# sunshinnnn/DSMnet

Hardware: AMD Instinct MI355X
Metric: stereo pairs/sec forward, PSMNet D=192 384×1280, at 1/2/4/8 MI355X (higher is better)
Workload: dtype f32

## Files before the change

dsmnet_amd/_lib.py:

```python
import ctypes
import os

_HERE = os.path.dirname(os.path.abspath(__file__))
LIB_PATH = os.environ.get("DSM_LIB_PATH") or os.path.join(_HERE, "csrc", "libdsmnet_hip.so")

c_int, c_void_p, c_size_t = ctypes.c_int, ctypes.c_void_p, ctypes.c_size_t

DSM_OK = 0
DSM_F32 = 0
DSM_NCDHW, DSM_NDHWC = 0, 1
DSM_CONV_FP32_MFMA, DSM_CONV_COUT1_CHUNKED, DSM_CONV_TM_SHIFT, DSM_CONV_BLOCKS_SHIFT = 1, 2, 4, 16
DSM_CONV_NO_NSPLIT = 4
DSM_CONV_NO_ONCE = 8
DSM_CONV_KSPLIT_SHIFT = 8
DSM_PREC_F32, DSM_PREC_F16, DSM_PREC_F16X2 = 0, 1, 2
DSM_SIM_DOT, DSM_SIM_COSINE = 0, 1
DSM_CORR_BWD_NAIVE = 1


class Bn3dArgs(ctypes.Structure):
    _fields_ = [("y", c_void_p), ("residual", c_void_p), ("out", c_void_p), ("gamma", c_void_p),
                ("beta", c_void_p), ("running_mean", c_void_p), ("running_var", c_void_p),
                ("affine", c_void_p), ("workspace", c_void_p), ("gout", c_void_p), ("dy", c_void_p),
                ("dresidual", c_void_p), ("B", c_int), ("C", c_int),
                ("Dy", c_int), ("Hy", c_int), ("Wy", c_int), ("Dr", c_int), ("Hr", c_int), ("Wr", c_int),
                ("relu", c_int), ("momentum", ctypes.c_float), ("eps", ctypes.c_float),
                ("out_amax", c_void_p), ("dy_amax", c_void_p), ("dres_amax", c_void_p)]


class Conv3dArgs(ctypes.Structure):
    _fields_ = [("x", c_void_p), ("w_packed", c_void_p), ("scale", c_void_p),
                ("shift", c_void_p), ("residual", c_void_p), ("y", c_void_p),
                ("B", c_int), ("Cin", c_int), ("Cout", c_int),
                ("Di", c_int), ("Hi", c_int), ("Wi", c_int),
                ("Do", c_int), ("Ho", c_int), ("Wo", c_int),
                ("Dr", c_int), ("Hr", c_int), ("Wr", c_int),
                ("stride", c_int), ("transposed", c_int), ("relu", c_int),
                ("kd", c_int), ("k", c_int), ("dil", c_int),
                ("flags", c_int), ("precision", c_int), ("x_amax", c_void_p), ("y_amax", c_void_p),
                ("vol_virtual", c_int), ("vol_mask_left", c_int),
                ("workspace", c_void_p), ("workspace_bytes", c_size_t)]
# ... 135 lines not shown
    "dsm_conv_packed_weight_bytes": (ctypes.c_size_t, [c_int] * 4),
    "dsm_spp_branch_floats": (ctypes.c_size_t, [c_int] * 3),
    "dsm_spp_pool8": (c_int, [c_void_p] * 2 + [c_int] * 3 + [c_void_p]),
    "dsm_spp_branches": (c_int, [c_void_p] * 5 + [c_int] * 3 + [c_void_p]),
    "dsm_spp_concat": (c_int, [c_void_p] * 4 + [c_int] * 3 + [c_void_p] * 2),
    "dsm_warp_abs_error": (c_int, [c_void_p] * 4 + [c_int] * 6 + [ctypes.c_float, c_void_p]),
    "dsm_warp_abs_error_bwd": (c_int, [c_void_p] * 7 + [c_int] * 6 + [ctypes.c_float, c_void_p]),
    "dsm_decoder_cat_bwd": (c_int, [c_void_p] * 6 + [c_int] * 11 + [c_void_p]),
    "dsm_selfsup_workspace_floats": (c_size_t, [ctypes.POINTER(SelfsupItem), c_int]),
    "dsm_selfsup_fwd": (c_int, [ctypes.POINTER(SelfsupItem), c_int, c_int] + [c_void_p] * 4),
    "dsm_selfsup_bwd": (c_int, [ctypes.POINTER(SelfsupItem), c_int, c_int] + [c_void_p] * 4),
    "dsm_selfsup_ext_workspace_floats": (c_size_t, [ctypes.POINTER(SelfsupItem), c_int, c_int]),
    "dsm_selfsup_ext_fwd": (c_int, [ctypes.POINTER(SelfsupItem), ctypes.POINTER(SelfsupExt), c_int, c_int] + [c_void_p] * 4),
    "dsm_selfsup_ext_bwd": (c_int, [ctypes.POINTER(SelfsupItem), ctypes.POINTER(SelfsupExt), c_int, c_int] + [c_void_p] * 4),
    "dsm_selfsup_dyn_fwd": (c_int, [ctypes.POINTER(SelfsupItem), ctypes.POINTER(SelfsupExt), c_int, c_int] + [c_void_p] * 5),
    "dsm_selfsup_dyn_bwd": (c_int, [ctypes.POINTER(SelfsupItem), ctypes.POINTER(SelfsupExt), c_int, c_int] + [c_void_p] * 5),
    "dsm_suploss_workspace_floats": (c_size_t, [c_int] * 5),
    "dsm_suploss_fwd": (c_int, [ctypes.POINTER(SuplossItem), c_int, c_void_p, c_int, c_int, c_int, c_int] + [c_void_p] * 4),
    "dsm_suploss_bwd": (c_int, [ctypes.POINTER(SuplossItem), c_int, c_void_p, c_int, c_int, c_int] + [c_void_p] * 4),
    "dsm_stereo_metrics_workspace_bytes": (c_size_t, [c_int] * 3),
    "dsm_stereo_metrics": (c_int, [ctypes.POINTER(MetricsArgs), c_void_p]),
    "dsm_lr_check": (c_int, [ctypes.POINTER(LrcheckArgs), c_void_p]),
    "dsm_fill_background_workspace_bytes": (c_size_t, [c_int] * 3),
    "dsm_fill_background": (c_int, [c_void_p] * 4 + [c_int] * 3 + [c_void_p]),
    "dsm_disp_encode_workspace_bytes": (c_size_t, [c_int] * 3),
    "dsm_disp_encode": (c_int, [ctypes.POINTER(EncodeArgs), c_void_p]),
    "dsm_stereo_color": (c_int, [c_void_p, c_void_p, ctypes.POINTER(ColorRecord)] + [c_int] * 6 + [c_void_p]),
    "dsm_stereo_spatial": (c_int, [c_void_p, c_void_p, ctypes.POINTER(SpatialRecord)] + [c_int] * 8 + [c_void_p]),
    "dsm_stereo_spatial_raw": (c_int, [c_void_p, c_size_t, ctypes.POINTER(FrameSource), c_void_p,
                                       ctypes.POINTER(SpatialRecord)] + [c_int] * 8 + [c_void_p]),
    "dsm_stereo_spatial_raw_plan": (c_int, [c_void_p, c_size_t, ctypes.POINTER(FrameSource), c_void_p,
                                            ctypes.POINTER(SpatialRecord)] + [c_int] * 8),
    "dsm_concat_conv_fwd": (c_int, [c_void_p] * 5 + [c_size_t] + [c_void_p] * 2 + [c_int] * 9 + [c_void_p]),
}

_lib = None


class DsmnetHipError(RuntimeError):
    pass


def _bind_torch_hip_runtime():
    import torch
    hip = os.path.join(os.path.dirname(torch.__file__), "lib", "libamdhip64.so")
    if os.path.exists(hip):
        ctypes.CDLL(hip, mode=ctypes.RTLD_GLOBAL)


def load():
    global _lib
    if _lib is not None:
        return _lib
    if not os.path.exists(LIB_PATH):
        raise DsmnetHipError(
            "libdsmnet_hip.so not found at %s -- build it with "
            "`python -m dsmnet_amd.csrc.build` (there is no CPU fallback)" % LIB_PATH)
    _bind_torch_hip_runtime()
    lib = ctypes.CDLL(LIB_PATH)
    for name, (res, args) in SIGNATURES.items():
        fn = getattr(lib, name)
        fn.restype = res
        fn.argtypes = args
    if lib.dsm_abi_version() != 7:
        raise DsmnetHipError("libdsmnet_hip.so ABI version mismatch")
    _lib = lib
# ... 8 lines not shown
```

dsmnet_amd/blocks2d.py:

```python
import torch
import torch.nn as nn
import torch.nn.functional as F

from . import costvolume as cv
from . import blocks3d
from .folds import _bump_running_stats, _versions, fold_affine

_TRAIN_2D_MODE = __import__("os").environ.get("DSM_TRAIN_2D", "auto")
_FUSED_TRAIN_2D = _TRAIN_2D_MODE in ("auto", "fused", "conv")
_FUSED_TRAIN_2D_BN = _TRAIN_2D_MODE == "fused"
_TRAIN_2D_MIN_PIXELS = int(__import__("os").environ.get("DSM_TRAIN_2D_MIN_PIXELS", 65536)) if _TRAIN_2D_MODE == "auto" else 0


class own_kernels_only(object):

    def __enter__(self):
        global _TRAIN_2D_MIN_PIXELS, _FUSED_TRAIN_2D
        self.saved = (_TRAIN_2D_MIN_PIXELS, _FUSED_TRAIN_2D)
        _TRAIN_2D_MIN_PIXELS, _FUSED_TRAIN_2D = 0, True
        return self

    def __exit__(self, *exc):
        global _TRAIN_2D_MIN_PIXELS, _FUSED_TRAIN_2D
        _TRAIN_2D_MIN_PIXELS, _FUSED_TRAIN_2D = self.saved
# ... 56 lines not shown
    if not (cv.get_option("wide_conv2d_train") and isinstance(act, nn.ReLU) and isinstance(conv, nn.Conv2d) and
            x.is_cuda and x.dtype == torch.float32):
        return False
    k, s, d, p = conv.kernel_size, conv.stride, conv.dilation, conv.padding
    if k != (3, 3) or s[0] != s[1] or s[0] not in (1, 2) or d != (1, 1) or p != (1, 1) or conv.groups != 1:
        return False
    if conv.bias is None or conv.padding_mode != "zeros" or conv.weight.dtype != torch.float32:
        return False
    if conv.in_channels not in cv.WIDE2D_COUT or conv.out_channels not in cv.WIDE2D_COUT:
        return False
    B, _, H, W = x.shape
    Ho, Wo = (H - 1) // s[0] + 1, (W - 1) // s[0] + 1
    if W > 2032 or B * H * W >= 2 ** 20 or 4 * B * Ho * Wo * conv.out_channels >= 2 ** 31:
        return False
    return _wide_ok(conv, x)


class _Folded2d(object):
    def __init__(self):
        self.key = None
        self.packed = self.scale = self.shift = None

    def get(self, conv, bn, cin_padded):
        srcs = [conv.weight, conv.bias]
        if bn is not None:
            srcs += [bn.weight, bn.bias, bn.running_mean, bn.running_var]
        key = _versions(*srcs) + (cin_padded,)
        if key != self.key:
            with torch.no_grad():
                self.packed = cv.pack_conv2d_weight(conv.weight, cin_padded)
                self.scale, self.shift = fold_affine(conv.bias, bn, conv.out_channels, conv.weight.device)
            self.key = key
        return self.packed, self.scale, self.shift


def train_ok(conv, x):
    if not (_FUSED_TRAIN_2D and isinstance(conv, nn.Conv2d) and torch.is_tensor(x) and x.is_cuda and
            x.dtype == torch.float32 and conv.weight.dtype == torch.float32):
        return False
    k, s, d, p = conv.kernel_size, conv.stride, conv.dilation, conv.padding
    if k[0] != k[1] or s[0] != s[1] or d[0] != d[1] or p[0] != p[1] or conv.groups != 1:
        return False
    if conv.bias is not None or conv.padding_mode != "zeros" or p[0] != d[0] * (k[0] // 2):
        return False
    if x.shape[0] * ((x.shape[2] - 1) // s[0] + 1) * ((x.shape[3] - 1) // s[0] + 1) < _TRAIN_2D_MIN_PIXELS:
        return False
    return x.shape[1] == conv.in_channels and cv.conv2d_variant(conv.out_channels, s[0], k[0], d[0])


def _run_conv2d_autograd(conv, bn, x, residual, relu):
    y = cv.conv2d(x, conv.weight, conv.stride[0], conv.dilation[0])
    if (bn is not None and bn.training and _FUSED_TRAIN_2D_BN and blocks3d._FUSED_TRAIN_BN and
            y.shape[1] % 4 == 0 and y.shape[1] <= 256):
        momentum = bn.momentum if bn.momentum is not None else 0.1
        out = cv.bn_add_relu2d(y, bn.weight, bn.bias, residual,
                               bn.running_mean if bn.track_running_stats else None,
                               bn.running_var if bn.track_running_stats else None,
                               1 if relu else 0, momentum, bn.eps)
        if bn.num_batches_tracked is not None:
            bn.num_batches_tracked += 1
        _bump_running_stats(bn)
        return out
    if bn is not None:
        y = bn(y)
    if residual is not None:
        y = y + residual
    return F.relu(y) if relu else y


def run_conv2d(folded, conv, bn, x, residual=None, relu=False):
    training = bn is not None and bn.training
    if not training and not torch.is_grad_enabled() and fused_ok(conv, x):
        packed, scale, shift = folded.get(conv, bn, x.shape[1])
        return cv.conv2d_block(x, packed, conv.out_channels, scale, shift, residual,
                               stride=conv.stride[0], relu=1 if relu else 0,
                               k=conv.kernel_size[0], dilation=conv.dilation[0])
    if train_ok(conv, x):
        return _run_conv2d_autograd(conv, bn, x, residual, relu)
    if x.shape[1] != conv.in_channels:
        x = x[:, : conv.in_channels]
    y = conv(x)
    if bn is not None:
        y = bn(y)
    if residual is not None:
        y = y + residual
    return F.relu(y) if relu else y


def run_basicblock_layers(fold1, c1, b1, fold2, c2, b2, x, relu_after, skip=True):
    if b1 is None or b2 is None or c1.training or b1.training or b2.training or torch.is_grad_enabled():
        return None
    if not (fused_ok(c1, x) and fused_ok(c2, x) and c1.kernel_size[0] == 3 and c2.kernel_size[0] == 3 and
            c2.stride[0] == 1 and c2.dilation[0] == 1 and c2.in_channels == c2.out_channels == c1.out_channels and
            cv.basicblock2d_ok(x, c1.in_channels, c1.out_channels, c1.stride[0], c1.dilation[0])):
        return None
    p1, s1, h1 = fold1.get(c1, b1, x.shape[1])
    p2, s2, h2 = fold2.get(c2, b2, x.shape[1])
    return cv.basicblock2d(x, p1, s1, h1, p2, s2, h2, relu=relu_after, skip=skip)


def run_basicblock(cb1, cb2, x, downsample):
    if downsample is not None or not isinstance(cb1, ConvBN2d) or not isinstance(cb2, ConvBN2d):
        return None
    return run_basicblock_layers(cb1._folded, cb1[0], cb1[1], cb2._folded, cb2[0], cb2[1], x, False)

# ... 14 lines not shown
```

dsmnet_amd/costvolume.py:

```python
import collections
import ctypes
import functools
import os
import weakref

import torch

from . import _lib
from .folds import _versions

_CL3D = torch.channels_last_3d


class LaunchTimer(object):

    def __init__(self):
        self.records = []

    def start(self):
        ev = torch.cuda.Event(enable_timing=True)
        ev.record()
        return ev

    def stop(self, name, start, work):
# ... 446 lines not shown
            setattr(a, field, 16)
    buf = ctypes.create_string_buffer(96)
    rc = _lib.load().dsm_conv3d_plan(ctypes.byref(a), buf, 96)
    return rc, buf.value.decode()


_PRECISIONS = ("bf16x3", "fp32", "f16x2", "f16")


def _env_precision():
    v = os.environ.get("DSM_CONV_PRECISION", "")
    if v and v not in _PRECISIONS:
        raise ValueError("DSM_CONV_PRECISION must be one of %s, got %r" % (_PRECISIONS, v))
    return v or "f16x2"


def _env_flag(name, default):
    v = os.environ.get(name, "")
    if v not in ("", "0", "1"):
        raise ValueError("%s must be 0 or 1, got %r" % (name, v))
    return default if v == "" else v == "1"


_WIDE_CONV2D_DEFAULT = False

_OPTIONS = {"fuse_volume": True, "fuse_blocks": True, "conv_precision": _env_precision(), "conv_flags": 0,
            "separable_volume": _env_flag("DSM_SEPARABLE_VOLUME", True), "separable_flags": 0,
            "fused_supervised_loss": _env_flag("DSM_FUSED_SUP_LOSS", True),
            "wide_conv2d": _env_flag("DSM_WIDE_CONV2D", _WIDE_CONV2D_DEFAULT),
            "wide_conv2d_train": _env_flag("DSM_WIDE_CONV2D_TRAIN", False),
            "conv2d_k5": _env_flag("DSM_CONV2D_K5", False),
            "warp_train": _env_flag("DSM_WARP_TRAIN", False),
            "decoder_train": _env_flag("DSM_DECODER_TRAIN", False),
            "corr1d_tiled_bwd": False}


def set_option(name, value):
    if name == "conv_fp32":
        old = _OPTIONS["conv_precision"] == "fp32"
        _OPTIONS["conv_precision"] = "fp32" if value else "bf16x3"
        return old
    if name not in _OPTIONS:
        raise KeyError(name)
    old = _OPTIONS[name]
    if name == "conv_precision":
        if value not in _PRECISIONS:
            raise ValueError("conv_precision must be one of %s" % (_PRECISIONS,))
        _OPTIONS[name] = value
    else:
        _OPTIONS[name] = int(value) if name in ("conv_flags", "separable_flags") else bool(value)
    return old


def _mode(mode):
    return _OPTIONS["conv_precision"] if mode is None else mode


def _conv_flags(mode=None):
    return (_lib.DSM_CONV_FP32_MFMA if _mode(mode) == "fp32" else 0) | _OPTIONS["conv_flags"]


def get_option(name):
    if name == "conv_fp32":
        return _OPTIONS["conv_precision"] == "fp32"
    return _OPTIONS[name]

# ... 623 lines not shown
        if needs_amax():
            dy._dsm_amax = _ARENA.slot(y.device)
            a.dy_amax = dy._dsm_amax.data_ptr()
            if dres is not None:
                dres._dsm_amax = _ARENA.slot(y.device)
                a.dres_amax = dres._dsm_amax.data_ptr()
        with torch.cuda.device(y.device), _timed("bn3d_train_bwd_kernels", 4.0 * (3 * y.numel() + gout.numel())):
            rc = _lib.load().dsm_bn3d_train_bwd(ctypes.byref(a), _stream())
        _lib.check(rc, "dsm_bn3d_train_bwd")
        dbeta = ws[:C].float() if has_beta else None
        dgamma = ws[C:].float() if has_gamma else None
        return dy, dgamma, dbeta, dres, None, None, None, None, None


def bn_add_relu3d(y, gamma, beta, residual, running_mean, running_var, relu, momentum, eps):
    return BnAddRelu3dFunction.apply(y, gamma, beta, residual, running_mean, running_var, int(relu),
                                     float(momentum), float(eps))


def stage_images_nhwc16(left, right=None):
    _require_device("stage_images_nhwc16", left, right)
    left = left.contiguous()
    B, C, H, W = left.shape
    if right is not None:
        if tuple(right.shape) != tuple(left.shape):
            raise ValueError("stage_images_nhwc16: the two views differ in shape")
        right = right.contiguous()
    out = torch.empty(((1 if right is None else 2) * B, 16, H, W), device=left.device,
                      dtype=torch.float32, memory_format=_CL2D)
    with torch.cuda.device(left.device):
        rc = _lib.load().dsm_stage_images_nhwc16(_p(left), _p(right), _p(out), B, C, H, W, _stream())
    _lib.check(rc, "dsm_stage_images_nhwc16")
    return out


def conv2d_variant(cout, stride, k, dilation):
    if cout not in (32, 64, 128) or k not in (1, 3) or stride < 1 or dilation < 1:
        return False
    return _conv2d_variant(cout, stride, k, dilation, _mode(None), _conv_flags())


@functools.lru_cache(maxsize=None)
def _conv2d_variant(cout, stride, k, dilation, mode, flags):
    return _conv_plan(_conv2d_standin(1, 16, cout, 12, 40, stride, k, dilation, mode, flags))[0] == _lib.DSM_OK


def _wgrad2d(x_cl, g_cl, stride, dilation, label="conv2d_wgrad_kernel", mode=None):
    B, cx, Hx, Wx = x_cl.shape
    _, cg, Hg, Wg = g_cl.shape
    ws = torch.empty((cx // 32) * (cg // 32) * 9 * 1024, device=x_cl.device, dtype=torch.float32)
    dw = torch.empty((cg, cx, 3, 3), device=x_cl.device, dtype=torch.float32)
    prec, xa, ga = _wgrad_precision(x_cl, g_cl, mode)
    with torch.cuda.device(x_cl.device), _timed(label, 18.0 * cx * cg * B * Hg * Wg):
        rc = _lib.load().dsm_conv2d_wgrad(_p(x_cl), _p(g_cl), _p(ws), _p(dw), B, cx, cg, Hx, Wx,
                                          Hg, Wg, int(stride), int(dilation), _conv_flags(mode), prec,
                                          _p(xa), _p(ga), _stream())
    _lib.check(rc, "dsm_conv2d_wgrad")
    return dw


class Conv2dFunction(torch.autograd.Function):

    @staticmethod
    def forward(ctx, x, weight, stride, dilation):
        _require_device("Conv2dFunction", x, weight)
        cout, cin, k, _ = weight.shape
# ... 838 lines not shown
```

dsmnet_amd/csrc/build.py:

```python
import glob
import os
import subprocess
import sys
from concurrent.futures import ThreadPoolExecutor

HERE = os.path.dirname(os.path.abspath(__file__))
SOURCES = ["abi.hip", "corr1d.hip", "cost_volume.hip", "soft_argmin.hip", "conv3d.hip", "conv_f16.hip",
           "conv3d_bwd.hip", "bn3d.hip", "decoder.hip", "spp.hip", "warp.hip",
           "selfsup.hip", "color.hip", "spatial.hip", "frames.hip", "sepvol.hip", "suploss.hip", "relu_bwd.hip",
           "metrics.hip", "lrcheck.hip", "encode.hip"]
LIB = os.path.join(HERE, "libdsmnet_hip.so")
HIPCC = os.environ.get("HIPCC", "/opt/rocm/bin/hipcc")
FLAGS = ["--offload-arch=gfx950", "-O3", "-std=c++17", "-fPIC",
         "-Wall", "-Wno-unused-function"] + os.environ.get("HIPCC_EXTRA", "").split()


def _stale(out, deps):
    if not os.path.exists(out):
        return True
    t = os.path.getmtime(out)
    return any(os.path.getmtime(d) > t for d in deps)


def build(force=False, verbose=True, stamps=False):
    if stamps:
        lib = os.path.join(HERE, "libdsmnet_hip_stamps.so")
        srcs = [os.path.join(HERE, s) for s in SOURCES]
        extra = ["-DDSM_ABLATE=%s" % os.environ["DSM_ABLATE"]] if os.environ.get("DSM_ABLATE") else []
        cmd = [HIPCC] + FLAGS + ["-DDSM_STAMPS"] + extra + ["-shared", "-o", lib] + srcs
        print(" ".join(cmd), flush=True)
        subprocess.run(cmd, check=True)
        return lib
    hdrs = sorted(glob.glob(os.path.join(HERE, "*.hpp"))) + [os.path.join(HERE, "..", "..", "include", "dsmnet_hip.h")]
    srcs = [os.path.join(HERE, s) for s in SOURCES if os.path.exists(os.path.join(HERE, s))]
    objs = []
    jobs = []
    for s in srcs:
        o = s[:-4] + ".o"
        objs.append(o)
        if force or _stale(o, [s] + hdrs):
            jobs.append([HIPCC] + FLAGS + ["-c", s, "-o", o])

    def run(cmd):
# ... 18 lines not shown
```

dsmnet_amd/models/psmnet/stackhourglass.py:

```python
import math

import torch
import torch.nn as nn

from ... import costvolume as cv
from ...blocks3d import Chain3d, ConvBN3d
from .submodule import convbn_3d, disparityregression, feature_extraction


def myadd_3d(tensor1, tensor2):
    assert tensor1.dim() == 5
    d, h, w = (min(a, b) for a, b in zip(tensor1.shape[2:], tensor2.shape[2:]))
    return tensor1[:, :, :d, :h, :w] + tensor2[:, :, :d, :h, :w]


def _deconvbn_3d(cin, cout):
    return ConvBN3d(nn.ConvTranspose3d(cin, cout, kernel_size=3, padding=1, output_padding=1,
                                       stride=2, bias=False), nn.BatchNorm3d(cout))


class hourglass(nn.Module):
    def __init__(self, inplanes):
        super(hourglass, self).__init__()
        c = inplanes
# ... 19 lines not shown
        self.name = "psmnet"
        self.maxdisp = maxdisp
        self.align_corners = bool(align_corners)
        self.count_levels = 1
        self.feature_extraction = feature_extraction(align_corners=align_corners)
        relu = lambda: nn.ReLU(inplace=True)
        self.dres0 = Chain3d(convbn_3d(64, 32, 3, 1, 1), relu(), convbn_3d(32, 32, 3, 1, 1), relu())
        self.dres1 = Chain3d(convbn_3d(32, 32, 3, 1, 1), relu(), convbn_3d(32, 32, 3, 1, 1))
        self.dres2 = hourglass(32)
        self.dres3 = hourglass(32)
        self.dres4 = hourglass(32)
        for i in (1, 2, 3):
            setattr(self, "classif%d" % i, Chain3d(
                convbn_3d(32, 32, 3, 1, 1), relu(),
                nn.Conv3d(32, 1, kernel_size=3, padding=1, stride=1, bias=False)))
        self._init_weights()

    def _init_weights(self):
        for m in self.modules():
            if isinstance(m, (nn.Conv2d, nn.Conv3d)):
                fan = m.out_channels
                for k in m.kernel_size:
                    fan *= k
                m.weight.data.normal_(0, math.sqrt(2.0 / fan))
            elif isinstance(m, (nn.BatchNorm2d, nn.BatchNorm3d)):
                m.weight.data.fill_(1)
                m.bias.data.zero_()

    def features(self, left, right):
        if self.training:
            return self.feature_extraction(left), self.feature_extraction(right)
        fe = self.feature_extraction
        if left.is_cuda and not torch.is_grad_enabled() and left.shape[1] <= 16:
            both = fe(cv.stage_images_nhwc16(left, right), staged=True)
        else:
            both = self.feature_extraction(torch.cat([left, right], dim=0))
        self.__dict__["_both"] = both
        return (cv.carry_amax(both[: left.shape[0]], both), cv.carry_amax(both[left.shape[0]:], both))

    def regularise(self, cost):
        cost0 = self.dres0(cost)
        cost0 = self.dres1(cost0, residual=cost0)
        out1, pre1, post1 = self.dres2(cost0, None, None, skip=cost0)
        out2, pre2, post2 = self.dres3(out1, pre1, post1, skip=cost0)
        out3, pre3, post3 = self.dres4(out2, pre1, post2, skip=cost0)
        cost1 = self.classif1(out1)
        cost2 = self.classif2(out2, residual=cost1)
        cost3 = self.classif3(out3, residual=cost2)
        return cost1, cost2, cost3

    def forward(self, left, right, mode="train"):
        with cv.amax_scope(left.device):
            return self._forward(left, right)

    def head_cost(self, left, right):
        if self.training:
            raise RuntimeError("PSMNet.head_cost: eval mode only (call model.eval() first)")
        with cv.amax_scope(left.device):
            (_, _, cost3), size = self._head_costs(left, right)
        return cost3, size, False, self.align_corners, None

    def _forward(self, left, right):
        (cost1, cost2, cost3), size = self._head_costs(left, right)
        pred1 = cv.soft_argmin(cost1, size, align_corners=self.align_corners)
        pred2 = cv.soft_argmin(cost2, size, align_corners=self.align_corners)
        pred3 = cv.soft_argmin(cost3, size, align_corners=self.align_corners)
        return [0, 0, 0], [pred3, pred2, pred1]
# ... 13 lines not shown
```

dsmnet_amd/models/psmnet/submodule.py:

```python
import torch
import torch.nn as nn
import torch.nn.functional as F

from ... import blocks2d
from ... import costvolume as cv
from ...blocks2d import ConvBN2d, _Folded2d, run_conv2d, stage_image_nhwc16
from ...blocks3d import ConvBN3d
from ...folds import _versions, fold_affine

_SPP_MATMUL = __import__("os").environ.get("DSM_TRAIN_SPP", "matmul") != "interp"
_TRAIN_NHWC = __import__("os").environ.get("DSM_TRAIN_LAYOUT", "nchw") == "nhwc"


def convbn(in_planes, out_planes, kernel_size, stride, pad, dilation):
    del pad
    return ConvBN2d(
        nn.Conv2d(in_planes, out_planes, kernel_size=kernel_size, stride=stride,
                  padding=dilation, dilation=dilation, bias=False),
        nn.BatchNorm2d(out_planes))


def convbn_3d(in_planes, out_planes, kernel_size, stride, pad):
    conv = nn.Conv3d(in_planes, out_planes, kernel_size=kernel_size, padding=pad,
                     stride=stride, bias=False)
# ... 84 lines not shown
            return F.interpolate(y, size=size, mode="bilinear", align_corners=self.align_corners)
        key = (y.shape[2], y.shape[3], size[0], size[1], self.align_corners, y.device)
        cache = self.__dict__.setdefault("_up_cache", {})
        if key not in cache:
            cache[key] = (self._bilinear_matrix(y.shape[2], size[0], self.align_corners, y.device),
                          self._bilinear_matrix(y.shape[3], size[1], self.align_corners, y.device).t().contiguous())
        ry, rxt = cache[key]
        return torch.matmul(ry, torch.matmul(y.contiguous(), rxt))

    def _spp_stock(self, raw, skip):
        size = skip.shape[2:]
        pooled, pyramid = skip, []
        for i in (4, 3, 2, 1):
            pooled = F.avg_pool2d(pooled, 8 if i == 4 else 2)
            branch = getattr(self, "branch%d" % i)
            y = branch[1](pooled, relu=True)
            pyramid.append(self._upsample(y, size))
        return torch.cat([raw, skip] + pyramid, dim=1)

    def _spp_params(self):
        convs = [getattr(self, "branch%d" % i)[1] for i in (4, 3, 2, 1)]
        srcs = [t for c in convs for t in (c[0].weight, c[1].weight, c[1].bias,
                                           c[1].running_mean, c[1].running_var)]
        key = _versions(*srcs)
        if getattr(self, "_spp_key", None) != key:
            with torch.no_grad():
                w_t = torch.stack([c[0].weight.reshape(32, 128).t() for c in convs]).contiguous()
                rows = [fold_affine(None, c[1], 32, c[0].weight.device) for c in convs]
                scale, shift = (torch.stack(r) for r in zip(*rows))
            self._spp_cache = (w_t, scale, shift)
            self._spp_key = key
        return self._spp_cache

    def forward(self, x, staged=False):
        fast = x.is_cuda and not self.training and not torch.is_grad_enabled()
        if staged and not fast:
            raise RuntimeError("feature_extraction: staged input exists on the eval fast path only")
        if fast and not staged:
            x = stage_image_nhwc16(x)
        elif _TRAIN_NHWC and x.is_cuda:
            x = x.contiguous(memory_format=torch.channels_last)
        x = self.firstconv[0](x, relu=True)
        fc2, fc4 = self.firstconv[2], self.firstconv[4]
        y = blocks2d.run_basicblock_layers(fc2._folded, fc2[0], fc2[1], fc4._folded, fc4[0], fc4[1], x, True, skip=False)
        x = y if y is not None else fc4(fc2(x, relu=True), relu=True)
        x = self.layer1(x)
        raw = self.layer2(x)
        skip = self.layer4(self.layer3(raw))
        if skip.is_cuda and not self.training and not torch.is_grad_enabled() and not self.align_corners:
            x = cv.spp_head(raw, skip, *self._spp_params())
        else:
            x = self._spp_stock(raw, skip)
        x = self.lastconv[0](x, relu=True)
        if not hasattr(self, "_last_fold"):
            self._last_fold = _Folded2d()
        return run_conv2d(self._last_fold, self.lastconv[2], None, x)
```

include/dsmnet_hip.h:

```cpp
#ifndef DSMNET_HIP_H
#define DSMNET_HIP_H

#include <stddef.h>
#include <stdint.h>

#ifdef __cplusplus
extern "C" {
#endif

#define DSM_ABI_VERSION 7

#define DSM_OK               0
#define DSM_ERR_ARG         -1
#define DSM_ERR_UNSUPPORTED -2
#define DSM_ERR_LAUNCH      -3
#define DSM_ERR_ALIGN       -4

enum dsm_dtype  { DSM_F32 = 0 };
enum dsm_layout { DSM_NCDHW = 0, DSM_NDHWC = 1 };

typedef void* dsm_stream_t;

int         dsm_abi_version(void);
const char* dsm_strerror(int code);
// ... 358 lines not shown
  double scale_x, scale_y;
} dsm_spatial_record;

int dsm_stereo_spatial(const void* x, void* y, const dsm_spatial_record* recs, int n_recs, int B, int C,
                       int H0, int W0, int h, int w, int to_tensor_channels, dsm_stream_t stream);

#define DSM_DISP_F32 0
#define DSM_DISP_U16_256 1
#define DSM_DISP_U16 2
#define DSM_DISP_U8 3
#define DSM_FRAMES_MAX_RECORDS 32
typedef struct dsm_frame_source {
  long long imL, imR;
  long long dispL, dispR;
  int Hs, Ws;
  int y0, x0;
  int flip;
  int disp_format;
  int pad_[2];
} dsm_frame_source;

int dsm_stereo_spatial_raw(const void* raw, size_t raw_bytes, const dsm_frame_source* srcs, void* y,
                           const dsm_spatial_record* recs, int n_recs, int B, int C, int H0, int W0, int h,
                           int w, int to_tensor_channels, dsm_stream_t stream);
int dsm_stereo_spatial_raw_plan(const void* raw, size_t raw_bytes, const dsm_frame_source* srcs, void* y,
                                const dsm_spatial_record* recs, int n_recs, int B, int C, int H0, int W0,
                                int h, int w, int to_tensor_channels);

int dsm_concat_conv_fwd(const void* both, const void* w_packed, const void* scale, const void* shift,
                        void* workspace, size_t workspace_floats, void* y, float* y_amax,
                        int B, int C, int Cout, int D, int H, int W,
                        int mask_left, int relu, int flags, dsm_stream_t stream);

#ifdef __cplusplus
}
#endif
#endif
```

Before: 215.4.

## Add direct NCHW stride-2 stem conv kernel and MFMA pointwise 1x1 conv path

Adds a dedicated kernel that reads the raw NCHW left/right images and computes the first 3x3 stride-2 conv with folded BN and ReLU, writing NHWC output directly. This skips the separate NHWC16 staging pass and the padded generic first conv, and it is enabled by default. It also adds an fp32-MFMA 1x1 pointwise conv kernel for the 2D tower, but that path is off by default behind an env flag. The stem kernel uses plain FMAs with strided global loads, so its efficiency relative to the padded generic conv is uncertain.

```diff
diff --git a/dsmnet_amd/_lib.py b/dsmnet_amd/_lib.py
--- a/dsmnet_amd/_lib.py
+++ b/dsmnet_amd/_lib.py
@@ -7,6 +7,7 @@
 c_int, c_void_p, c_size_t = ctypes.c_int, ctypes.c_void_p, ctypes.c_size_t
 
 DSM_OK = 0
+DSM_ERR_UNSUPPORTED = -2
 DSM_F32 = 0
 DSM_NCDHW, DSM_NDHWC = 0, 1
 DSM_CONV_FP32_MFMA, DSM_CONV_COUT1_CHUNKED, DSM_CONV_TM_SHIFT, DSM_CONV_BLOCKS_SHIFT = 1, 2, 4, 16
@@ -208,6 +209,8 @@
     "dsm_stereo_spatial_raw_plan": (c_int, [c_void_p, c_size_t, ctypes.POINTER(FrameSource), c_void_p,
                                             ctypes.POINTER(SpatialRecord)] + [c_int] * 8),
     "dsm_concat_conv_fwd": (c_int, [c_void_p] * 5 + [c_size_t] + [c_void_p] * 2 + [c_int] * 9 + [c_void_p]),
+    "dsm_stem_s2_fwd": (c_int, [c_void_p] * 7 + [c_int] * 4 + [c_void_p]),
+    "dsm_pointwise2d_fwd": (c_int, [c_void_p] * 6 + [c_int] * 8 + [c_void_p]),
 }
 
 _lib = None
diff --git a/dsmnet_amd/blocks2d.py b/dsmnet_amd/blocks2d.py
--- a/dsmnet_amd/blocks2d.py
+++ b/dsmnet_amd/blocks2d.py
@@ -112,6 +112,18 @@
                 self.scale, self.shift = fold_affine(conv.bias, bn, conv.out_channels, conv.weight.device)
             self.key = key
         return self.packed, self.scale, self.shift
+
+    def get_seam(self, conv, bn, pack):
+        srcs = [conv.weight, conv.bias]
+        if bn is not None:
+            srcs += [bn.weight, bn.bias, bn.running_mean, bn.running_var]
+        key = _versions(*srcs) + (pack.__name__,)
+        if key != self.__dict__.get("seam_key"):
+            with torch.no_grad():
+                weight = pack(conv.weight)
+                scale, shift = fold_affine(conv.bias, bn, conv.out_channels, conv.weight.device)
+            self.seam, self.seam_key = (weight, scale, shift), key
+        return self.seam
 
 
 def train_ok(conv, x):
@@ -151,6 +163,13 @@
 def run_conv2d(folded, conv, bn, x, residual=None, relu=False):
     training = bn is not None and bn.training
     if not training and not torch.is_grad_enabled() and fused_ok(conv, x):
+        if (conv.kernel_size[0] == 1 and residual is None and x.shape[1] == conv.in_channels and
+                cv.get_option("pointwise_1x1")):
+            packed, scale, shift = folded.get_seam(conv, bn, cv.pack_pointwise_weight)
+            y = cv.pointwise2d_block(x, packed, conv.out_channels, scale, shift, stride=conv.stride[0],
+                                     relu=1 if relu else 0)
+            if y is not None:
+                return y
         packed, scale, shift = folded.get(conv, bn, x.shape[1])
         return cv.conv2d_block(x, packed, conv.out_channels, scale, shift, residual,
                                stride=conv.stride[0], relu=1 if relu else 0,
diff --git a/dsmnet_amd/costvolume.py b/dsmnet_amd/costvolume.py
--- a/dsmnet_amd/costvolume.py
+++ b/dsmnet_amd/costvolume.py
@@ -502,6 +502,8 @@
             "conv2d_k5": _env_flag("DSM_CONV2D_K5", False),
             "warp_train": _env_flag("DSM_WARP_TRAIN", False),
             "decoder_train": _env_flag("DSM_DECODER_TRAIN", False),
+            "direct_stem": _env_flag("DSM_DIRECT_STEM", True),
+            "pointwise_1x1": _env_flag("DSM_POINTWISE_1X1", False),
             "corr1d_tiled_bwd": False}
 
 
@@ -1191,6 +1193,74 @@
         rc = _lib.load().dsm_stage_images_nhwc16(_p(left), _p(right), _p(out), B, C, H, W, _stream())
     _lib.check(rc, "dsm_stage_images_nhwc16")
     return out
+
+
+SEAM_CHANNELS = (32, 64, 128)
+
+
+def pack_stem_weight(weight):
+    if tuple(weight.shape) != (32, 3, 3, 3):
+        raise ValueError("pack_stem_weight: a (32,3,3,3) weight, got %s" % (tuple(weight.shape),))
+    return weight.detach().permute(1, 2, 3, 0).reshape(27, 32).contiguous()
+
+
+def pack_pointwise_weight(weight):
+    cout, cin = weight.shape[:2]
+    if tuple(weight.shape[2:]) != (1, 1) or cin % 8 or cout % 32:
+        raise ValueError("pack_pointwise_weight: a (Cout,Cin,1,1) weight with Cin %% 8 == 0 and Cout %% 32 == 0, got %s"
+                         % (tuple(weight.shape),))
+    w = weight.detach().reshape(cout // 32, 32, 2, cin // 8, 4)
+    return w.permute(0, 3, 2, 1, 4).contiguous().reshape(-1)
+
+
+def stem_s2_block(left, right, packed_weight, scale=None, shift=None, relu=True):
+    _require_device("stem_s2_block", left, right, packed_weight, scale, shift)
+    if left.dim() != 4 or left.shape[1] != 3 or left.dtype != torch.float32:
+        raise ValueError("stem_s2_block: (B,3,H,W) float32 images, got %s %s" % (tuple(left.shape), left.dtype))
+    left = left.contiguous()
+    B, _, H, W = left.shape
+    if right is not None:
+        if tuple(right.shape) != tuple(left.shape) or right.dtype != torch.float32:
+            raise ValueError("stem_s2_block: the two views differ in shape or dtype")
+        right = right.contiguous()
+    N = B if right is None else 2 * B
+    Ho, Wo = (H - 1) // 2 + 1, (W - 1) // 2 + 1
+    y = torch.empty((N, 32, Ho, Wo), device=left.device, dtype=torch.float32, memory_format=_CL2D)
+    ya = _ARENA.slot(y.device) if needs_amax() else None
+    work = 4.0 * (N * 3 * H * W + y.numel() + packed_weight.numel())
+    with torch.cuda.device(left.device), _timed("conv2d_stem_s2_kernel", work):
+        rc = _lib.load().dsm_stem_s2_fwd(_p(left), _p(right), _p(packed_weight), _p(scale), _p(shift), _p(y), _p(ya),
+                                         B, H, W, 1 if relu else 0, _stream())
+    _lib.check(rc, "dsm_stem_s2_fwd")
+    if ya is not None:
+        y._dsm_amax = ya
+    return y
+
+
+def pointwise2d_block(x, packed_weight, cout, scale=None, shift=None, stride=1, relu=0, grid=0):
+    _require_device("pointwise2d_block", x, packed_weight, scale, shift)
+    if not x.is_contiguous(memory_format=_CL2D):
+        x = carry_amax(x.contiguous(memory_format=_CL2D), x)
+    B, cin, Hi, Wi = x.shape
+    stride = int(stride)
+    if stride < 1:
+        raise ValueError("pointwise2d_block: stride %d" % stride)
+    Ho, Wo = (Hi - 1) // stride + 1, (Wi - 1) // stride + 1
+    y = torch.empty((B, cout, Ho, Wo), device=x.device, dtype=torch.float32, memory_format=_CL2D)
+    ya = _ARENA.slot(y.device) if needs_amax() else None
+    work = 4.0 * (B * Ho * Wo * cin + y.numel() + cin * cout)
+    with torch.cuda.device(x.device):
+        t0 = _timer.start() if _timer is not None else None
+        rc = _lib.load().dsm_pointwise2d_fwd(_p(x), _p(packed_weight), _p(scale), _p(shift), _p(y), _p(ya),
+                                             B, cin, cout, Hi, Wi, stride, 1 if relu else 0, int(grid), _stream())
+        if rc == _lib.DSM_ERR_UNSUPPORTED:
+            return None
+        _lib.check(rc, "dsm_pointwise2d_fwd")
+        if t0 is not None:
+            _timer.stop("conv2d_pointwise_kernel<%d,%d,%d>" % (cin, cout, stride), t0, work)
+    if ya is not None:
+        y._dsm_amax = ya
+    return y
 
 
 def conv2d_variant(cout, stride, k, dilation):
diff --git a/dsmnet_amd/csrc/build.py b/dsmnet_amd/csrc/build.py
--- a/dsmnet_amd/csrc/build.py
+++ b/dsmnet_amd/csrc/build.py
@@ -8,7 +8,7 @@
 SOURCES = ["abi.hip", "corr1d.hip", "cost_volume.hip", "soft_argmin.hip", "conv3d.hip", "conv_f16.hip",
            "conv3d_bwd.hip", "bn3d.hip", "decoder.hip", "spp.hip", "warp.hip",
            "selfsup.hip", "color.hip", "spatial.hip", "frames.hip", "sepvol.hip", "suploss.hip", "relu_bwd.hip",
-           "metrics.hip", "lrcheck.hip", "encode.hip"]
+           "metrics.hip", "lrcheck.hip", "encode.hip", "towers_seams.hip"]
 LIB = os.path.join(HERE, "libdsmnet_hip.so")
 HIPCC = os.environ.get("HIPCC", "/opt/rocm/bin/hipcc")
 FLAGS = ["--offload-arch=gfx950", "-O3", "-std=c++17", "-fPIC",
diff --git a/dsmnet_amd/csrc/towers_seams.hip b/dsmnet_amd/csrc/towers_seams.hip
--- /dev/null
+++ b/dsmnet_amd/csrc/towers_seams.hip
@@ -0,0 +1,280 @@
+#include "split_core.hpp"
+
+namespace {
+
+constexpr int ST_CO = 32;
+
+struct StemArgs {
+  const float* left; const float* right; const float* wp; const float* scale; const float* shift;
+  float* y; float* y_amax;
+  int B, H, W, Ho, Wo, relu;
+};
+
+__global__ __launch_bounds__(256) void conv2d_stem_s2_kernel(StemArgs p) {
+  __shared__ f32x4 wl[27 * 8];
+  __shared__ f32x4 aff[16];
+  __shared__ float red[4];
+  const int lane = threadIdx.x & 63, wave = threadIdx.x >> 6;
+  const int xo = blockIdx.x * 64 + lane, yo = blockIdx.y * 8 + wave * 2, n = blockIdx.z;
+  const bool col = xo < p.Wo;
+  const float* src = (n < p.B ? p.left + (long)n * 3 * p.H * p.W : p.right + (long)(n - p.B) * 3 * p.H * p.W);
+
+  if (threadIdx.x < 27 * 8) {
+    wl[threadIdx.x] = reinterpret_cast<const f32x4*>(p.wp)[threadIdx.x];
+  } else if (threadIdx.x < 27 * 8 + 16) {
+    const int i = threadIdx.x - 27 * 8;
+    const float fill = i < 8 ? 1.f : 0.f;
+    f32x4 a = {fill, fill, fill, fill};
+    if (p.scale) {
+      const float* s = i < 8 ? p.scale + 4 * i : p.shift + 4 * (i - 8);
+      a = f32x4{s[0], s[1], s[2], s[3]};
+    }
+    aff[i] = a;
+  }
+
+  auto fetch = [&](int it, float (&d)[2][3]) {
+    const int c = it / 3, ky = it - 3 * c;
+#pragma unroll
+    for (int r = 0; r < 2; ++r)
+#pragma unroll
+      for (int kx = 0; kx < 3; ++kx) {
+        const int yy = 2 * (yo + r) - 1 + ky, xx = 2 * xo - 1 + kx;
+        const bool ok = col && yy >= 0 && yy < p.H && xx >= 0 && xx < p.W;
+        d[r][kx] = ok ? src[((long)c * p.H + yy) * p.W + xx] : 0.f;
+      }
+  };
+  float nxt[2][3];
+  fetch(0, nxt);
+  __syncthreads();
+
+  f32x4 acc[2][8];
+#pragma unroll
+  for (int r = 0; r < 2; ++r)
+#pragma unroll
+    for (int q = 0; q < 8; ++q) acc[r][q] = f32x4{0.f, 0.f, 0.f, 0.f};
+#pragma unroll 1
+  for (int it = 0; it < 9; ++it) {
+    float cur[2][3];
+#pragma unroll
+    for (int r = 0; r < 2; ++r)
+#pragma unroll
+      for (int kx = 0; kx < 3; ++kx) cur[r][kx] = nxt[r][kx];
+    if (it + 1 < 9) fetch(it + 1, nxt);
+#pragma unroll
+    for (int kx = 0; kx < 3; ++kx)
+#pragma unroll
+      for (int q = 0; q < 8; ++q) {
+        const f32x4 w4 = wl[(it * 3 + kx) * 8 + q];
+#pragma unroll
+        for (int r = 0; r < 2; ++r)
+#pragma unroll
+          for (int i = 0; i < 4; ++i) acc[r][q][i] = fmaf(cur[r][kx], w4[i], acc[r][q][i]);
+      }
+  }
+
+  float am = 0.f;
+#pragma unroll
+  for (int r = 0; r < 2; ++r) {
+    if (col && yo + r < p.Ho) {
+      f32x4* dst = reinterpret_cast<f32x4*>(p.y + (((long)n * p.Ho + yo + r) * p.Wo + xo) * ST_CO);
+#pragma unroll
+      for (int q = 0; q < 8; ++q) {
+        const f32x4 sc = aff[q], sh = aff[8 + q];
+        f32x4 s;
+#pragma unroll
+        for (int i = 0; i < 4; ++i) {
+          const float e = fmaf(acc[r][q][i], sc[i], sh[i]);
+          s[i] = p.relu ? fmaxf(e, 0.f) : e;
+        }
+        track_amax(am, s);
+        dst[q] = s;
+      }
+    }
+  }
+  publish_amax<4, false>(p.y_amax, am, red);
+}
+
+struct PwArgs {
+  const float* x; const float* wp; const float* scale; const float* shift;
+  float* y; float* y_amax;
+  long M;
+  int Hi, Wi, Ho, Wo, stride, relu;
+};
+
+template <int CIN>
+__device__ __forceinline__ void pw_load(const PwArgs& p, long g, long ngroups, int lane, f32x4 (&raw)[CIN / 8]) {
+  constexpr int C4 = CIN / 4;
+#pragma unroll
+  for (int q = 0; q < CIN / 8; ++q) {
+    const int chunk = q * 64 + lane;
+    const long m = g * 32 + chunk / C4;
+    const bool ok = g < ngroups && m < p.M;
+    long in = ok ? m : 0;
+    if (p.stride != 1) {
+      const unsigned hw = (unsigned)p.Ho * (unsigned)p.Wo, mm = (unsigned)in;
+      const unsigned n = mm / hw, r = mm - n * hw;
+      const unsigned yo = r / (unsigned)p.Wo, xo = r - yo * (unsigned)p.Wo;
+      in = ((long)n * p.Hi + (long)yo * p.stride) * p.Wi + (long)xo * p.stride;
+    }
+    const f32x4* src = reinterpret_cast<const f32x4*>(p.x + in * CIN + (chunk % C4) * 4);
+    raw[q] = ok ? *src : f32x4{0.f, 0.f, 0.f, 0.f};
+  }
+}
+
+__device__ __forceinline__ void pw_wave_sync() {
+  __builtin_amdgcn_fence(__ATOMIC_RELEASE, "wavefront");
+  __builtin_amdgcn_wave_barrier();
+  __builtin_amdgcn_fence(__ATOMIC_ACQUIRE, "wavefront");
+}
+
+template <int CIN> constexpr int pw_occupancy() { return CIN == 128 ? 1 : 2; }
+template <int CIN, int COUT> constexpr size_t pw_lds_bytes() { return ((size_t)CIN * COUT + 4 * 32 * (CIN + 4)) * 4; }
+
+template <int CIN, int COUT>
+__global__ __launch_bounds__(256, (pw_occupancy<CIN>())) void conv2d_pointwise_kernel(PwArgs p) {
+  constexpr int T = COUT / 32, J4 = CIN / 8, C4 = CIN / 4, ROW = CIN + 4;
+  extern __shared__ __align__(16) float pw_lds[];
+  __shared__ float red[4];
+  f32x4* wl = reinterpret_cast<f32x4*>(pw_lds);
+  const int lane = threadIdx.x & 63, wave = threadIdx.x >> 6;
+  float* tile = pw_lds + CIN * COUT + wave * (32 * ROW);
+  const int pix = lane & 31, h = lane >> 5;
+  const long ngroups = (p.M + 31) >> 5;
+  const long gstride = (long)gridDim.x * 4;
+  long g = (long)blockIdx.x * 4 + wave;
+
+  f32x4 raw[J4];
+  pw_load<CIN>(p, g, ngroups, lane, raw);
+  {
+    constexpr int NW = CIN * COUT / 4 / 256;
+    const f32x4* wsrc = reinterpret_cast<const f32x4*>(p.wp);
+    f32x4 wreg[NW];
+#pragma unroll
+    for (int i = 0; i < NW; ++i) wreg[i] = wsrc[i * 256 + threadIdx.x];
+#pragma unroll
+    for (int i = 0; i < NW; ++i) wl[i * 256 + threadIdx.x] = wreg[i];
+  }
+  float sc[T], sh[T];
+#pragma unroll
+  for (int t = 0; t < T; ++t) {
+    sc[t] = p.scale ? p.scale[t * 32 + pix] : 1.f;
+    sh[t] = p.scale ? p.shift[t * 32 + pix] : 0.f;
+  }
+  __syncthreads();
+
+  float am = 0.f;
+  for (; g < ngroups; g += gstride) {
+#pragma unroll
+    for (int q = 0; q < J4; ++q) {
+      const int chunk = q * 64 + lane;
+      *reinterpret_cast<f32x4*>(tile + (chunk / C4) * ROW + (chunk % C4) * 4) = raw[q];
+    }
+    pw_wave_sync();
+    f32x4 a[J4];
+#pragma unroll
+    for (int j = 0; j < J4; ++j) a[j] = *reinterpret_cast<const f32x4*>(tile + pix * ROW + h * (CIN / 2) + 4 * j);
+    pw_wave_sync();
+    pw_load<CIN>(p, g + gstride, ngroups, lane, raw);
+    float* dst = p.y + (g * 32) * COUT + pix;
+#pragma unroll
+    for (int t = 0; t < T; ++t) {
+      f32x16 acc = {0.f, 0.f, 0.f, 0.f, 0.f, 0.f, 0.f, 0.f, 0.f, 0.f, 0.f, 0.f, 0.f, 0.f, 0.f, 0.f};
+#pragma unroll
+      for (int j = 0; j < J4; ++j) {
+        const f32x4 w4 = wl[(t * J4 + j) * 64 + lane];
+        acc = __builtin_amdgcn_mfma_f32_32x32x2f32(a[j].x, w4.x, acc, 0, 0, 0);
+        acc = __builtin_amdgcn_mfma_f32_32x32x2f32(a[j].y, w4.y, acc, 0, 0, 0);
+        acc = __builtin_amdgcn_mfma_f32_32x32x2f32(a[j].z, w4.z, acc, 0, 0, 0);
+        acc = __builtin_amdgcn_mfma_f32_32x32x2f32(a[j].w, w4.w, acc, 0, 0, 0);
+      }
+#pragma unroll
+      for (int r = 0; r < 16; ++r) {
+        const int row = (r & 3) + 8 * (r >> 2) + 4 * h;
+        float v = acc[r];
+        if (p.scale) v = fmaf(v, sc[t], sh[t]);
+        if (p.relu) v = fmaxf(v, 0.f);
+        if (g * 32 + row < p.M) {
+          am = fmaxf(am, fabsf(v));
+          dst[(long)row * COUT + t * 32] = v;
+        }
+      }
+    }
+  }
+  publish_amax<4, false>(p.y_amax, am, red);
+}
+
+template <int CIN, int COUT>
+int pw_launch(const PwArgs& p, int forced, hipStream_t s) {
+  constexpr size_t lds = pw_lds_bytes<CIN, COUT>();
+  const long ngroups = (p.M + 31) / 32;
+  long blocks = (ngroups + 3) / 4;
+  const long cap = forced ? forced : 256 * pw_occupancy<CIN>();
+  blocks = blocks < cap ? blocks : cap;
+  const int rc = dsm_allow_lds<conv2d_pointwise_kernel<CIN, COUT>>(lds);
+  if (rc != DSM_OK) return rc;
+  dsm_clear_stale_error();
+  hipLaunchKernelGGL((conv2d_pointwise_kernel<CIN, COUT>), dim3((unsigned)blocks), dim3(256), lds, s, p);
+  return dsm_launch_status();
+}
+
+template <int CIN>
+int pw_launch_cout(const PwArgs& p, int Cout, int forced, hipStream_t s) {
+  switch (Cout) {
+    case 32: return pw_launch<CIN, 32>(p, forced, s);
+    case 64: return pw_launch<CIN, 64>(p, forced, s);
+    case 128: return pw_launch<CIN, 128>(p, forced, s);
+  }
+  return DSM_ERR_UNSUPPORTED;
+}
+
+inline bool seam_channels(int c) { return c == 32 || c == 64 || c == 128; }
+
+}
+
+extern "C" int dsm_stem_s2_fwd(const void* left, const void* right, const void* w_packed, const void* scale,
+                               const void* shift, void* y, float* y_amax, int B, int H, int W, int relu,
+                               dsm_stream_t stream) {
+  DSM_REQUIRE(left && w_packed && y, DSM_ERR_ARG);
+  DSM_REQUIRE((scale == nullptr) == (shift == nullptr), DSM_ERR_ARG);
+  DSM_REQUIRE(B >= 1 && H >= 1 && W >= 1, DSM_ERR_ARG);
+  DSM_REQUIRE(dsm_aligned16(y) && dsm_aligned16(w_packed) && (((uintptr_t)left | (uintptr_t)right | (uintptr_t)scale |
+                                    (uintptr_t)shift | (uintptr_t)y_amax) & 3u) == 0, DSM_ERR_ALIGN);
+  const int N = right ? 2 * B : B;
+  const int Ho = (H - 1) / 2 + 1, Wo = (W - 1) / 2 + 1;
+  DSM_REQUIRE(B <= 32767 && dsm_cdiv(Ho, 8) <= 65535 && (long)3 * H * W < (1L << 31), DSM_ERR_UNSUPPORTED);
+  StemArgs p;
+  p.left = (const float*)left; p.right = (const float*)right; p.wp = (const float*)w_packed;
+  p.scale = (const float*)scale; p.shift = (const float*)shift;
+  p.y = (float*)y; p.y_amax = y_amax;
+  p.B = B; p.H = H; p.W = W; p.Ho = Ho; p.Wo = Wo; p.relu = relu ? 1 : 0;
+  dsm_clear_stale_error();
+  hipLaunchKernelGGL(conv2d_stem_s2_kernel, dim3((unsigned)dsm_cdiv(Wo, 64), (unsigned)dsm_cdiv(Ho, 8), (unsigned)N),
+                     dim3(256), 0, (hipStream_t)stream, p);
+  return dsm_launch_status();
+}
+
+extern "C" int dsm_pointwise2d_fwd(const void* x, const void* w_packed, const void* scale, const void* shift,
+                                   void* y, float* y_amax, int B, int Cin, int Cout, int Hi, int Wi, int stride,
+                                   int relu, int flags, dsm_stream_t stream) {
+  DSM_REQUIRE(x && w_packed && y, DSM_ERR_ARG);
+  DSM_REQUIRE((scale == nullptr) == (shift == nullptr), DSM_ERR_ARG);
+  DSM_REQUIRE(B >= 1 && Cin >= 1 && Cout >= 1 && Hi >= 1 && Wi >= 1 && stride >= 1 && flags >= 0, DSM_ERR_ARG);
+  DSM_REQUIRE(seam_channels(Cin) && seam_channels(Cout) && stride <= 2, DSM_ERR_UNSUPPORTED);
+  DSM_REQUIRE(dsm_aligned16(x) && dsm_aligned16(w_packed) && dsm_aligned16(y) &&
+              (((uintptr_t)scale | (uintptr_t)shift | (uintptr_t)y_amax) & 3u) == 0, DSM_ERR_ALIGN);
+  const int Ho = (Hi - 1) / stride + 1, Wo = (Wi - 1) / stride + 1;
+  const long M = (long)B * Ho * Wo;
+  DSM_REQUIRE(M < (1L << 31) && (long)B * Hi * Wi < (1L << 31), DSM_ERR_UNSUPPORTED);
+  PwArgs p;
+  p.x = (const float*)x; p.wp = (const float*)w_packed; p.scale = (const float*)scale; p.shift = (const float*)shift;
+  p.y = (float*)y; p.y_amax = y_amax;
+  p.M = M; p.Hi = Hi; p.Wi = Wi; p.Ho = Ho; p.Wo = Wo; p.stride = stride; p.relu = relu ? 1 : 0;
+  const int forced = flags & 0xffff;
+  hipStream_t s = (hipStream_t)stream;
+  switch (Cin) {
+    case 32: return pw_launch_cout<32>(p, Cout, forced, s);
+    case 64: return pw_launch_cout<64>(p, Cout, forced, s);
+    case 128: return pw_launch_cout<128>(p, Cout, forced, s);
+  }
+  return DSM_ERR_UNSUPPORTED;
+}
diff --git a/dsmnet_amd/models/psmnet/stackhourglass.py b/dsmnet_amd/models/psmnet/stackhourglass.py
--- a/dsmnet_amd/models/psmnet/stackhourglass.py
+++ b/dsmnet_amd/models/psmnet/stackhourglass.py
@@ -75,7 +75,11 @@
             return self.feature_extraction(left), self.feature_extraction(right)
         fe = self.feature_extraction
         if left.is_cuda and not torch.is_grad_enabled() and left.shape[1] <= 16:
-            both = fe(cv.stage_images_nhwc16(left, right), staged=True)
+            stem = fe.direct_stem(left, right) if tuple(right.shape) == tuple(left.shape) else None
+            if stem is not None:
+                both = fe(stem, stemmed=True)
+            else:
+                both = fe(cv.stage_images_nhwc16(left, right), staged=True)
         else:
             both = self.feature_extraction(torch.cat([left, right], dim=0))
         self.__dict__["_both"] = both
diff --git a/dsmnet_amd/models/psmnet/submodule.py b/dsmnet_amd/models/psmnet/submodule.py
--- a/dsmnet_amd/models/psmnet/submodule.py
+++ b/dsmnet_amd/models/psmnet/submodule.py
@@ -140,15 +140,29 @@
             self._spp_key = key
         return self._spp_cache
 
-    def forward(self, x, staged=False):
+    def direct_stem(self, left, right=None):
+        cb = self.firstconv[0]
+        if not (cv.get_option("direct_stem") and left.is_cuda and not self.training and not cb[1].training and
+                not torch.is_grad_enabled() and left.dim() == 4 and left.shape[1] == 3 and
+                left.dtype == torch.float32 and cb[0].weight.dtype == torch.float32):
+            return None
+        packed, scale, shift = cb._folded.get_seam(cb[0], cb[1], cv.pack_stem_weight)
+        return cv.stem_s2_block(left, right, packed, scale, shift, relu=True)
+
+    def forward(self, x, staged=False, stemmed=False):
         fast = x.is_cuda and not self.training and not torch.is_grad_enabled()
-        if staged and not fast:
+        if (staged or stemmed) and not fast:
             raise RuntimeError("feature_extraction: staged input exists on the eval fast path only")
-        if fast and not staged:
-            x = stage_image_nhwc16(x)
-        elif _TRAIN_NHWC and x.is_cuda:
+        if fast and not staged and not stemmed:
+            y = self.direct_stem(x)
+            if y is not None:
+                x, stemmed = y, True
+            else:
+                x = stage_image_nhwc16(x)
+        elif _TRAIN_NHWC and x.is_cuda and not stemmed:
             x = x.contiguous(memory_format=torch.channels_last)
-        x = self.firstconv[0](x, relu=True)
+        if not stemmed:
+            x = self.firstconv[0](x, relu=True)
         fc2, fc4 = self.firstconv[2], self.firstconv[4]
         y = blocks2d.run_basicblock_layers(fc2._folded, fc2[0], fc2[1], fc4._folded, fc4[0], fc4[1], x, True, skip=False)
         x = y if y is not None else fc4(fc2(x, relu=True), relu=True)
diff --git a/include/dsmnet_hip.h b/include/dsmnet_hip.h
--- a/include/dsmnet_hip.h
+++ b/include/dsmnet_hip.h
@@ -414,6 +414,14 @@
                         int B, int C, int Cout, int D, int H, int W,
                         int mask_left, int relu, int flags, dsm_stream_t stream);
 
+int dsm_stem_s2_fwd(const void* left, const void* right, const void* w_packed, const void* scale,
+                    const void* shift, void* y, float* y_amax, int B, int H, int W, int relu,
+                    dsm_stream_t stream);
+
+int dsm_pointwise2d_fwd(const void* x, const void* w_packed, const void* scale, const void* shift,
+                        void* y, float* y_amax, int B, int Cin, int Cout, int Hi, int Wi, int stride,
+                        int relu, int flags, dsm_stream_t stream);
+
 #ifdef __cplusplus
 }
 #endif
```

Result: no change. 216.7 (median of 6 runs) (+0.6%).
